# nextpyp/cet_pick

Hardware: AMD Instinct MI355X
Metric: subtomograms/sec (MoCo-3D train) + voxels/sec (heatmap+NMS) at 1/2/4/8 GPU (higher is better)
Workload: dtype f32; 1 GPU; moco_main.py moco3d_18: 3D encoder, synthetic 512x512x128 tomogram, 32^3 subtomo crops, batch 64 per GPU, r=1024, dim=128, m=0.999, T=0.1, SGD lr 1e-3; global_batch=64, parallelism=dp1, hipgraph=True

## Files before the change

cet_pick_amd/csrc/conv_direct3.hip:

```cpp
#include "common.h"
#include "bf16x3.h"
#include <type_traits>
#include <algorithm>

namespace {

using namespace bf3;

constexpr int C = 64;
constexpr int PLANE = 64;
constexpr int TZ = 2;
constexpr int PZ = TZ + 2;
constexpr int NV = PZ * PLANE;
constexpr int LEAD = 16;
constexpr int ZREC = 34;
constexpr int NREC = LEAD + NV + ZREC;
constexpr int ARR = NREC * 16;
constexpr int KS = C / 16;
constexpr int PL_BYTES = 2 * ARR;
constexpr int KS_BYTES = 3 * PL_BYTES;
constexpr int LDS_BYTES = KS * KS_BYTES;
constexpr int ZBASE = (LEAD + NV) * 16;
constexpr int WBLK = 1024;
constexpr int WSTEP = 2 * 3 * WBLK;
constexpr int NTAP = 27;
constexpr int NSTEP = KS * NTAP;
constexpr int WIMG_BYTES = NSTEP * WSTEP;
constexpr int RB = 6;
static_assert(NSTEP % RB == 0, "ring slots");
static_assert(LDS_BYTES <= 160 * 1024, "patch must fit the CU's LDS");
static_assert(((LEAD + NV) & 15) == 0, "zero region must start at a record = 0 (mod 16)");

struct Direct3Params {
    const float* a;
    const unsigned char* wimg;
    float* out;
    const float* res;
    const float* mask;
    int relu;
    int N, D;
    unsigned a_bytes;
};

template <bool TWO, int CT = C>
__global__ __launch_bounds__(256, TWO ? 2 : 1) void direct3_kernel(Direct3Params p) {
    constexpr int KS = CT / 16, NSTEP = KS * NTAP;
    constexpr int NSLOT = TWO ? 2 : KS;
    static_assert(NSTEP % RB == 0, "ring slots");
    __shared__ __attribute__((aligned(16))) unsigned char patch[NSLOT * KS_BYTES];
    const int tid = threadIdx.x, lane = tid & 63, wave = tid >> 6;
    const int h = lane >> 5, l32 = lane & 31;
    const int tz = wave >> 1, cw = wave & 1;
    const int zb = blockIdx.x % (p.D / TZ), n = blockIdx.x / (p.D / TZ);
    const int z0 = zb * TZ;

    const int cb = blockIdx.y;
    const __amdgpu_buffer_rsrc_t wrs = rsrc(p.wimg, (CT / 64) * NSTEP * WSTEP);
    const int w_voff = cw * (3 * WBLK) + lane * 16;
    const int w_cb = cb * (NSTEP * WSTEP);
    bf16x8 bfr[RB][3];
    auto wload = [&](int g, auto SLOTc) {
        constexpr int SLOT = decltype(SLOTc)::value;
#pragma unroll
        for (int pl = 0; pl < 3; ++pl)
            bfr[SLOT][pl] = __builtin_bit_cast(bf16x8, __builtin_amdgcn_raw_buffer_load_b128(wrs, g < NSTEP ? w_voff + pl * WBLK : (int)0x80000000u, g < NSTEP ? w_cb + g * WSTEP : 0, 0));
    };
    auto wload_dyn = [&](int g) {
        switch (g % RB) {
            case 0: wload(g, std::integral_constant<int, 0>{}); break;
            case 1: wload(g, std::integral_constant<int, 1>{}); break;
            case 2: wload(g, std::integral_constant<int, 2>{}); break;
            case 3: wload(g, std::integral_constant<int, 3>{}); break;
            case 4: wload(g, std::integral_constant<int, 4>{}); break;
            default: wload(g, std::integral_constant<int, 5>{}); break;
        }
    };
#pragma unroll
    for (int g = 0; g < RB - 1; ++g) wload_dyn(g);

    const __amdgpu_buffer_rsrc_t ars = rsrc(p.a, p.a_bytes);
    unsigned st_off[2];
    int st_lds[2];
#pragma unroll
    for (int u = 0; u < 2; ++u) {
        const int q = tid + 256 * u, vox = q >> 1, hh = q & 1;
        const int z = z0 - 1 + (vox >> 6);
        const bool ok = (unsigned)z < (unsigned)p.D;
        st_off[u] = ok ? 4u * (unsigned)((((long)n * p.D + z) * PLANE + (vox & 63)) * CT + hh * 8) : 0x80000000u;
        st_lds[u] = hh * ARR + (LEAD + vox) * 16;
    }
    u32x4 ld[2][2];
    auto stage_load = [&](int c) {
#pragma unroll
        for (int u = 0; u < 2; ++u) {
            ld[u][0] = __builtin_amdgcn_raw_buffer_load_b128(ars, (int)(st_off[u] + 64u * c), 0, 0);
            ld[u][1] = __builtin_amdgcn_raw_buffer_load_b128(ars, (int)(st_off[u] + 64u * c + 16u), 0, 0);
        }
    };
    auto stage_store = [&](int c) {
#pragma unroll
        for (int u = 0; u < 2; ++u) {
            float v[8];
#pragma unroll
            for (int e = 0; e < 4; ++e) { v[e] = __uint_as_float(ld[u][0][e]); v[4 + e] = __uint_as_float(ld[u][1][e]); }
            u32x4 o[3];
            cut8(v, o);
            unsigned char* dst = patch + (c % NSLOT) * KS_BYTES + st_lds[u];
#pragma unroll
            for (int pl = 0; pl < 3; ++pl) *reinterpret_cast<u32x4*>(dst + pl * PL_BYTES) = o[pl];
        }
    };
    stage_load(0);
    for (int i = tid; i < NSLOT * 3 * 2 * ZREC; i += 256) {
        const int arr = i / ZREC, r = i % ZREC;
        *reinterpret_cast<u32x4*>(patch + arr * ARR + ZBASE + r * 16) = u32x4{0u, 0u, 0u, 0u};
    }

    int vbase[2], zbase[2];
    unsigned vmask[2];
#pragma unroll
    for (int i = 0; i < 2; ++i) {
        const int y = 4 * i + (l32 >> 3), x = l32 & 7;
        const int rec = LEAD - 9 + tz * PLANE + y * 8 + x;
        vbase[i] = rec * 16 + h * ARR;
        zbase[i] = ZBASE + (rec & 15) * 16 + h * ARR;
        unsigned m = 0;
#pragma unroll
        for (int dy = 0; dy < 3; ++dy)
#pragma unroll
            for (int dx = 0; dx < 3; ++dx)
                if ((unsigned)(y + dy - 1) < 8u && (unsigned)(x + dx - 1) < 8u) m |= 1u << (dy * 3 + dx);
        vmask[i] = m;
    }

    f32x16 acc[2];
#pragma unroll
    for (int r = 0; r < 16; ++r) { acc[0][r] = 0.f; acc[1][r] = 0.f; }

    const long m0 = ((long)n * p.D + z0 + tz) * PLANE;
    const int col = cb * 64 + cw * 32 + l32;
    unsigned eoff[2][16];
    float rv[2][16], mv[2][16];
#pragma unroll
    for (int i = 0; i < 2; ++i)
#pragma unroll
        for (int r = 0; r < 16; ++r) eoff[i][r] = 4u * (unsigned)((m0 + 32 * i + (r & 3) + 8 * (r >> 2) + 4 * h) * CT + col);
    const __amdgpu_buffer_rsrc_t rrs = rsrc(p.res, p.res ? p.a_bytes : 0u), mrs = rsrc(p.mask, p.mask ? p.a_bytes : 0u);

    stage_store(0);
    stage_load(1);
    __syncthreads();

    bf16x8 af[2][2][3];
    int sel[9][2];
    auto make_sel = [&](int dz) {
#pragma unroll
        for (int t9 = 0; t9 < 9; ++t9)
#pragma unroll
            for (int i = 0; i < 2; ++i) sel[t9][i] = ((vmask[i] >> t9) & 1u) ? vbase[i] + dz * (PLANE * 16) : zbase[i];
    };
    auto frags = [&](int c, int t9, auto SETc) {
        constexpr int SET = decltype(SETc)::value;
        const int imm = ((t9 / 3) * 8 + (t9 % 3)) * 16 + (c % NSLOT) * KS_BYTES;
#pragma unroll
        for (int i = 0; i < 2; ++i)
#pragma unroll
            for (int pl = 0; pl < 3; ++pl)
                af[SET][i][pl] = *reinterpret_cast<const bf16x8*>(patch + sel[t9][i] + imm + pl * PL_BYTES);
    };
    auto frags_dyn = [&](int g, int c, int t9) {
        if (g & 1) frags(c, t9, std::integral_constant<int, 1>{});
        else frags(c, t9, std::integral_constant<int, 0>{});
    };

    make_sel(0);
    frags_dyn(0, 0, 0);
    __builtin_amdgcn_sched_barrier(0);
#pragma unroll
    for (int c = 0; c < KS; ++c) {
#pragma unroll
        for (int dz = 0; dz < 3; ++dz) {
#pragma unroll
            for (int t9 = 0; t9 < 9; ++t9) {
                const int g = c * NTAP + dz * 9 + t9;
                wload_dyn(g + RB - 1);
                if (dz == 1 && t9 == 0 && c + 1 < KS) {
                    stage_store(c + 1);
                    if (c + 2 < KS) stage_load(c + 2);
                }
                if (!TWO && c == KS - 1 && dz == 0 && t9 == 0) {
#pragma unroll
                    for (int i = 0; i < 2; ++i)
#pragma unroll
                        for (int r = 0; r < 16; ++r) {
                            rv[i][r] = __uint_as_float(__builtin_amdgcn_raw_buffer_load_b32(rrs, (int)eoff[i][r], 0, 0));
                            mv[i][r] = __uint_as_float(__builtin_amdgcn_raw_buffer_load_b32(mrs, (int)eoff[i][r], 0, 0));
                        }
                }
                if (g + 1 < NSTEP) {
                    const int c2 = (g + 1) / NTAP, r2 = (g + 1) % NTAP;
                    if (r2 == 0) __syncthreads();
                    if (r2 % 9 == 0) make_sel(r2 / 9);
                    frags_dyn(g + 1, c2, r2 % 9);
                }
#pragma unroll
                for (int pr = 0; pr < 6; ++pr) {
                    acc[0] = __builtin_amdgcn_mfma_f32_32x32x16_bf16(af[g & 1][0][PA[pr]], bfr[g % RB][PB[pr]], acc[0], 0, 0, 0);
                    acc[1] = __builtin_amdgcn_mfma_f32_32x32x16_bf16(af[g & 1][1][PA[pr]], bfr[g % RB][PB[pr]], acc[1], 0, 0, 0);
                }
#pragma unroll
                for (int k = 0; k < 6; ++k) {
                    __builtin_amdgcn_sched_group_barrier(0x008, 1, 0);
                    __builtin_amdgcn_sched_group_barrier(0x100, 1, 0);
                }
#pragma unroll
                for (int k = 0; k < 3; ++k) {
                    __builtin_amdgcn_sched_group_barrier(0x008, 1, 0);
                    __builtin_amdgcn_sched_group_barrier(0x020, 1, 0);
                }
                __builtin_amdgcn_sched_group_barrier(0x008, 3, 0);
                __builtin_amdgcn_sched_barrier(0);
            }
        }
    }

    const bool has_mask = p.mask != nullptr;
    if constexpr (TWO) {
#pragma unroll
        for (int i = 0; i < 2; ++i) {
            float rr[16], mm[16];
#pragma unroll
            for (int r = 0; r < 16; ++r) {
                const unsigned eo = 4u * (unsigned)((m0 + 32 * i + (r & 3) + 8 * (r >> 2) + 4 * h) * CT + col);
                rr[r] = __uint_as_float(__builtin_amdgcn_raw_buffer_load_b32(rrs, (int)eo, 0, 0));
                mm[r] = __uint_as_float(__builtin_amdgcn_raw_buffer_load_b32(mrs, (int)eo, 0, 0));
            }
#pragma unroll
            for (int r = 0; r < 16; ++r) {
                const unsigned eo = 4u * (unsigned)((m0 + 32 * i + (r & 3) + 8 * (r >> 2) + 4 * h) * CT + col);
                float v = acc[i][r] + rr[r];
                if (p.relu) v = fmaxf(v, 0.f);
                if (has_mask) v = (mm[r] > 0.f) ? v : 0.f;
                p.out[eo / 4] = v;
            }
        }
        return;
    }
#pragma unroll
    for (int i = 0; i < 2; ++i)
#pragma unroll
        for (int r = 0; r < 16; ++r) {
            float v = acc[i][r] + rv[i][r];
            if (p.relu) v = fmaxf(v, 0.f);
            if (has_mask) v = (mv[i][r] > 0.f) ? v : 0.f;
            p.out[eoff[i][r] / 4] = v;
        }
}

constexpr int HP = 10;
constexpr int H_NV = PZ * HP * HP;
constexpr int H_ARR = H_NV * 16;
constexpr int H_PL = 2 * H_ARR;
constexpr int H_KS = 3 * H_PL;
constexpr int H_UNITS = (2 * H_NV + 255) / 256;

struct Direct3hParams {
    const float* a;
    const unsigned char* wimg;
    float* out;
    const float* res;
    const float* mask;
    int relu;
    int N, D, H, W;
    unsigned a_bytes;
};

__global__ __launch_bounds__(256, 2) void direct3h_kernel(Direct3hParams p) {
    __shared__ __attribute__((aligned(16))) unsigned char patch[2 * H_KS];
    const int tid = threadIdx.x, lane = tid & 63, wave = tid >> 6;
    const int h = lane >> 5, l32 = lane & 31;
    const int tz = wave >> 1, cw = wave & 1;
    const int txn = (p.W + 7) / 8, tyn = (p.H + 7) / 8;
    int bi = blockIdx.x;
    const int bx = bi % txn; bi /= txn;
    const int by = bi % tyn; bi /= tyn;
    const int zb = bi % (p.D / TZ), n = bi / (p.D / TZ);
    const int z0 = zb * TZ, y0 = by * 8, x0 = bx * 8;

    const __amdgpu_buffer_rsrc_t wrs = rsrc(p.wimg, WIMG_BYTES);
    const int w_voff = cw * (3 * WBLK) + lane * 16;
    bf16x8 bfr[RB][3];
    auto wload = [&](int g, auto SLOTc) {
        constexpr int SLOT = decltype(SLOTc)::value;
#pragma unroll
        for (int pl = 0; pl < 3; ++pl)
            bfr[SLOT][pl] = __builtin_bit_cast(bf16x8, __builtin_amdgcn_raw_buffer_load_b128(wrs, g < NSTEP ? w_voff + pl * WBLK : (int)0x80000000u, g < NSTEP ? g * WSTEP : 0, 0));
    };
    auto wload_dyn = [&](int g) {
        switch (g % RB) {
            case 0: wload(g, std::integral_constant<int, 0>{}); break;
            case 1: wload(g, std::integral_constant<int, 1>{}); break;
            case 2: wload(g, std::integral_constant<int, 2>{}); break;
            case 3: wload(g, std::integral_constant<int, 3>{}); break;
            case 4: wload(g, std::integral_constant<int, 4>{}); break;
            default: wload(g, std::integral_constant<int, 5>{}); break;
        }
// ... 147 lines not shown
    constexpr int KSn = CT / 16;
    const int lane = idx & 63, cw = (idx >> 6) & 1, rest = idx >> 7, ks = rest % KSn, tap = (rest / KSn) % NTAP, cb = rest / (KSn * NTAP);
    if (cb >= CT / 64) return;
    const int nn = cb * 64 + cw * 32 + (lane & 31), k0 = ks * 16 + 8 * (lane >> 5);
    float v[8];
    if (dgrad) {
        ld8(w + ((long)(NTAP - 1 - tap) * CT + nn) * CT + k0, v);
    } else {
#pragma unroll
        for (int e = 0; e < 8; ++e) v[e] = w[((long)tap * CT + k0 + e) * CT + nn];
    }
    u32x4 o[3];
    cut8(v, o);
    unsigned char* dst = img + (long)(((cb * KSn + ks) * NTAP + tap) * 2 + cw) * (3 * WBLK) + lane * 16;
    store_planes(dst, WBLK, o);
}
__global__ __launch_bounds__(256) void direct3_prep_kernel(PrepBatch b) {
    const int fmt = b.wide[blockIdx.y], idx = blockIdx.x * 256 + threadIdx.x;
    if (fmt == 1) { if (blockIdx.x < PREP_BLOCKS_WIDE) direct3s_prep_body(b.w[blockIdx.y], b.img[blockIdx.y], b.dgrad[blockIdx.y], idx); }
    else if (fmt == 2) { if (blockIdx.x < PREP_BLOCKS_WIDE) direct3_prep_body<128>(b.w[blockIdx.y], b.img[blockIdx.y], b.dgrad[blockIdx.y], idx); }
    else if (fmt == 3) direct3s256_prep_body(b.w[blockIdx.y], b.img[blockIdx.y], b.dgrad[blockIdx.y], idx);
    else if (blockIdx.x < PREP_BLOCKS) direct3_prep_body<C>(b.w[blockIdx.y], b.img[blockIdx.y], b.dgrad[blockIdx.y], idx);
}

constexpr int WG_SPLITS = 28;
constexpr int WROW = 64;
constexpr int WHALF = (PLANE + 1) * WROW;
constexpr int WPL = 2 * WHALF;
constexpr int WOP = 3 * WPL;
constexpr int WBUF = 2 * WOP;
constexpr int WZERO = PLANE * WROW;

constexpr int WG_MAXPROB = 4;
struct Direct3WgradParams {
    const float* x[WG_MAXPROB];
    const float* dy[WG_MAXPROB];
    float* slabs[WG_MAXPROB];
    int N, D;
    unsigned bytes;
    int nprob, splits;
    int H, W;
};

constexpr int W_HB = 3 * 2 * 8 * 128;
template <bool V4, int CT, bool TILED = false>
__global__ __launch_bounds__(512, 2) void direct3_wgrad_kernel(Direct3WgradParams p) {
    __shared__ __attribute__((aligned(16))) unsigned char lds[2 * WBUF + (TILED ? 2 * W_HB : 16)];
    unsigned char* const halo = lds + 2 * WBUF;
    static_assert(!TILED || (!V4 && CT == 64), "tiled planes: the 64-channel geometry");
    constexpr int NBLK = CT / 64;
    const int tid = threadIdx.x, lane = tid & 63;
    const int wave = __builtin_amdgcn_readfirstlane(tid >> 6);
    const int h = lane >> 5, l32 = lane & 31, i16 = lane & 15, g16 = (lane >> 4) & 1;
    const int kh = wave >> 2, wm = (wave >> 1) & 1, wn = wave & 1;
    const int per_grp = p.nprob * p.splits;
    const int grp = blockIdx.x / per_grp, rem = blockIdx.x % per_grp;
    const int pb = rem / p.splits, split = rem % p.splits, stride = p.splits;
    const int pair = grp % 9, chb = grp / 9;
    const int ci0 = (chb / NBLK) * 64, co0 = (chb % NBLK) * 64;
    const int dz = pair / 3, dy = pair % 3;
    const int tiles_x = TILED ? p.W >> 3 : 1, tiles = TILED ? (p.H >> 3) * tiles_x : 1;
    const int n_planes = p.N * p.D * tiles;

    const __amdgpu_buffer_rsrc_t xrs = rsrc(p.x[pb], p.bytes), yrs = rsrc(p.dy[pb], p.bytes);
    const int st_vox = tid >> 3, st_cg = tid & 7;
    const unsigned st_src = TILED ? 4u * (unsigned)(((st_vox >> 3) * p.W + (st_vox & 7)) * C + st_cg * 8)
                                  : 4u * (unsigned)(st_vox * CT + st_cg * 8);
    const int h_side = tid >> 8, h_row = (tid >> 5) & 7, h_c2 = tid & 31;
    const unsigned x_ch = 4u * (unsigned)ci0, y_ch = 4u * (unsigned)co0;
    const int zsh = V4 ? 0 : dz - 1;
    const int st_lds = (st_cg >> 2) * WHALF + st_vox * WROW + (st_cg & 3) * 16;
    auto next_plane = [&](int from) {
        if (V4) return from < n_planes ? from : -1;
        for (int pi = from; pi < n_planes; pi += stride) {
            const int zi = (pi / tiles) % p.D + dz - 1;
            if ((unsigned)zi < (unsigned)p.D) return pi;
        }
        return -1;
    };
    u32x4 ldx[2], ldy[2];
    u32x2 ldh = {0u, 0u};
    unsigned u_y, u_x, u_h;
    auto unit_offsets = [&](int pi) {
        if (pi < 0) { u_y = u_x = u_h = 0x80000000u; return; }
        if (!TILED) {
            u_y = 4u * (unsigned)((long)pi * PLANE * CT) + y_ch + st_src;
            u_x = 4u * (unsigned)((long)(pi + zsh) * PLANE * CT) + x_ch + st_src;
            u_h = 0x80000000u;
            return;
        }
        const int pl = pi / tiles, t = pi % tiles, y0 = (t / tiles_x) * 8, x0 = (t % tiles_x) * 8;
        u_y = 4u * (unsigned)((((long)pl * p.H + y0) * p.W + x0) * C) + st_src;
        const int xr = y0 + (st_vox >> 3) + dy - 1;
        u_x = (unsigned)xr < (unsigned)p.H
                  ? 4u * (unsigned)((((long)(pl + dz - 1) * p.H + xr) * p.W + x0 + (st_vox & 7)) * C + st_cg * 8) : 0x80000000u;
        const int hr = y0 + h_row + dy - 1, hc = h_side ? x0 + 8 : x0 - 1;
        u_h = ((unsigned)hr < (unsigned)p.H && (unsigned)hc < (unsigned)p.W)
                  ? 4u * (unsigned)((((long)(pl + dz - 1) * p.H + hr) * p.W + hc) * C + 2 * h_c2) : 0x80000000u;
    };
    auto stage_load = [&](int pi) {
        unit_offsets(pi);
        ldx[0] = __builtin_amdgcn_raw_buffer_load_b128(xrs, (int)u_x, 0, 0);
        ldx[1] = __builtin_amdgcn_raw_buffer_load_b128(xrs, (int)(u_x + 16u), 0, 0);
        ldy[0] = __builtin_amdgcn_raw_buffer_load_b128(yrs, (int)u_y, 0, 0);
        ldy[1] = __builtin_amdgcn_raw_buffer_load_b128(yrs, (int)(u_y + 16u), 0, 0);
        if (TILED) ldh = __builtin_amdgcn_raw_buffer_load_b64(xrs, (int)u_h, 0, 0);
    };
    unsigned hcu[3];
    auto halo_cut = [&]() {
        const unsigned a1 = rest(ldh[0]), b1 = rest(ldh[1]), a2 = rest(a1), b2 = rest(b1);
        hcu[0] = pack2(ldh[1], ldh[0]);
        hcu[1] = pack2(b1, a1);
        hcu[2] = pack2(b2, a2);
    };
    auto halo_store = [&](int buf) {
#pragma unroll
        for (int pl = 0; pl < 3; ++pl)
            *reinterpret_cast<unsigned*>(halo + buf * W_HB + ((pl * 2 + h_side) * 8 + h_row) * 128 + h_c2 * 4) = hcu[pl];
    };
    auto stage_store_unit = [&](int buf, int op) {
        float v[8];
#pragma unroll
        for (int e = 0; e < 4; ++e) {
            v[e] = __uint_as_float(op ? ldy[0][e] : ldx[0][e]);
            v[4 + e] = __uint_as_float(op ? ldy[1][e] : ldx[1][e]);
        }
        u32x4 o[3];
        cut8(v, o);
        unsigned char* dst = lds + buf * WBUF + op * WOP + st_lds;
#pragma unroll
        for (int pl = 0; pl < 3; ++pl) *reinterpret_cast<u32x4*>(dst + pl * WPL) = o[pl];
        if (TILED && op == 0) { halo_cut(); halo_store(buf); }
    };

    const int q4 = i16 >> 2;
    const int coloff = (16 * g16 + 4 * (i16 & 3)) * 2;
    const int b_base = wn * WHALF + (2 * kh * 16 + 8 * h + q4) * WROW + coloff;
    int a_sel[2][2];
#pragma unroll
    for (int lk = 0; lk < 2; ++lk)
#pragma unroll
        for (int hi = 0; hi < 2; ++hi) {
            const int v = 16 * (2 * kh + lk) + 8 * h + 4 * hi + q4;
            if (V4) {
                const int zi = (v >> 4) + dz - 1, yi = ((v >> 2) & 3) + dy - 1;
                a_sel[lk][hi] = wm * WHALF + (((unsigned)zi < 4u && (unsigned)yi < 4u) ? ((zi * 4 + yi) * 4 + (v & 3)) * WROW : WZERO) + coloff;
            } else if (TILED) {
                a_sel[lk][hi] = wm * WHALF + v * WROW + coloff;
            } else {
                const int yi = (v >> 3) + dy - 1;
                a_sel[lk][hi] = wm * WHALF + ((unsigned)yi < 8u ? (yi * 8 + (v & 7)) * WROW : WZERO) + coloff;
            }
        }
    int h_off[2];
#pragma unroll
    for (int lk = 0; lk < 2; ++lk) h_off[lk] = (2 * (2 * kh + lk) + h) * 128 + (32 * wm + l32) * 2;
    unsigned hl[2][2][3];

    f32x16 acc[3];
#pragma unroll
    for (int t = 0; t < 3; ++t)
#pragma unroll
        for (int r = 0; r < 16; ++r) acc[t][r] = 0.f;

    for (int i = tid; i < 2 * 2 * 3 * 2 * (WROW / 16); i += 512) {
        const int img = i / (WROW / 16), c16 = i % (WROW / 16);
        *reinterpret_cast<u32x4*>(lds + img * WHALF + WZERO + c16 * 16) = u32x4{0u, 0u, 0u, 0u};
    }

    int cur = next_plane(split);
    int nxt = cur >= 0 ? next_plane(cur + stride) : -1;
    stage_load(cur);
    if (cur >= 0) { stage_store_unit(0, 0); stage_store_unit(0, 1); }
    stage_load(nxt);
    __syncthreads();

    bf16x8 af[2][3][3], bfg[2][3];
    auto read_piece = [&](int buf, int lk, int j, auto SETc) {
        constexpr int SET = decltype(SETc)::value;
        const unsigned char* xb = lds + buf * WBUF;
        if (j < 3) {
            const unsigned char* yb = xb + WOP + b_base + lk * 16 * WROW + j * WPL;
            const bf16x4 lo = __builtin_amdgcn_ds_read_tr16_b64_v4bf16((lds_bf16x4*)(yb));
            const bf16x4 hi = __builtin_amdgcn_ds_read_tr16_b64_v4bf16((lds_bf16x4*)(yb + 4 * WROW));
            bfg[SET][j] = __builtin_shufflevector(lo, hi, 0, 1, 2, 3, 4, 5, 6, 7);
        } else {
            const int pl = j - 3;
            const bf16x4 lo = __builtin_amdgcn_ds_read_tr16_b64_v4bf16((lds_bf16x4*)(xb + pl * WPL + a_sel[lk][0]));
            const bf16x4 hi = __builtin_amdgcn_ds_read_tr16_b64_v4bf16((lds_bf16x4*)(xb + pl * WPL + a_sel[lk][1]));
            af[SET][1][pl] = __builtin_shufflevector(lo, hi, 0, 1, 2, 3, 4, 5, 6, 7);
            if (TILED) {
#pragma unroll
                for (int sd = 0; sd < 2; ++sd)
                    hl[SET][sd][pl] = *reinterpret_cast<const unsigned short*>(halo + buf * W_HB + ((pl * 2 + sd) * 8) * 128 + h_off[lk]);
            }
        }
    };
    auto read_piece_dyn = [&](int buf, int lk, int j) {
        if (lk & 1) read_piece(buf, lk, j, std::integral_constant<int, 1>{});
        else read_piece(buf, lk, j, std::integral_constant<int, 0>{});
    };
    auto read_pair = [&](int buf, int lk, int i) {
        constexpr int BP[3] = {0, 2, 1}, AP[3] = {2, 0, 1};
        read_piece_dyn(buf, lk, BP[i]);
        read_piece_dyn(buf, lk, 3 + AP[i]);
    };
    auto derive = [&](int set, int dxv, int pl) {
        const u32x4 c = __builtin_bit_cast(u32x4, af[set][1][pl]);
        u32x4 o;
        if (dxv == 0) {
            o[0] = c[0] << 16;
#pragma unroll
            for (int j = 1; j < 4; ++j) o[j] = __builtin_amdgcn_alignbit(c[j], c[j - 1], 16);
            if (V4) o[2] &= HI16;
            if (TILED) o[0] |= hl[set][0][pl];
        } else {
#pragma unroll
            for (int j = 0; j < 3; ++j) o[j] = __builtin_amdgcn_alignbit(c[j + 1], c[j], 16);
            o[3] = c[3] >> 16;
            if (V4) o[1] &= 0x0000ffffu;
            if (TILED) o[3] |= hl[set][1][pl] << 16;
        }
        af[set][dxv][pl] = __builtin_bit_cast(bf16x8, o);
    };
    unsigned cu[3][8];
    auto cut_a = [&](int op, int e) {
        cu[0][e] = op ? ldy[e >> 2][e & 3] : ldx[e >> 2][e & 3];
        cu[1][e] = rest(cu[0][e]);
    };
    auto cut_b = [&](int e) { cu[2][e] = rest(cu[1][e]); };
    auto store_piece = [&](int buf, int op, int pl) {
        u32x4 o;
#pragma unroll
        for (int d = 0; d < 4; ++d) o[d] = pack2(cu[pl][2 * d + 1], cu[pl][2 * d]);
        *reinterpret_cast<u32x4*>(lds + buf * WBUF + op * WOP + st_lds + pl * WPL) = o;
    };

    int buf = 0;
    if (cur >= 0) {
#pragma unroll
        for (int i = 0; i < 3; ++i) read_pair(0, 0, i);
    }
    constexpr int DXO[3] = {1, 0, 2};
    while (cur >= 0) {
        const int nn = nxt >= 0 ? next_plane(nxt + stride) : -1;
        unit_offsets(nn);
        __builtin_amdgcn_sched_barrier(0);
#pragma unroll
        for (int lk = 0; lk < 2; ++lk) {
            const int op = lk;
#pragma unroll
            for (int m = 0; m < 18; ++m) {
                const int dxm = DXO[m / 6];
                acc[dxm] = __builtin_amdgcn_mfma_f32_32x32x16_bf16(af[lk][dxm][PA[m % 6]], bfg[lk][PB[m % 6]], acc[dxm], 0, 0, 0);
                if (m < 3) derive(lk, 0, m);
                if (m >= 6 && m < 9) derive(lk, 2, m - 6);
                if (m >= 2 && m < 10) cut_a(op, m - 2);
                if (m >= 3 && m < 11) cut_b(m - 3);
                if (m >= 11 && m < 14) store_piece(buf ^ 1, op, m - 11);
                if (lk == 1 && m >= 14) {
                    const int i = m - 14, hf = i & 1;
                    if (i < 2) ldx[hf] = __builtin_amdgcn_raw_buffer_load_b128(xrs, (int)(u_x + 16u * hf), 0, 0);
                    else ldy[hf] = __builtin_amdgcn_raw_buffer_load_b128(yrs, (int)(u_y + 16u * hf), 0, 0);
                    if (TILED && i == 3) ldh = __builtin_amdgcn_raw_buffer_load_b64(xrs, (int)u_h, 0, 0);
                }
                if (TILED && lk == 0 && m == 14) halo_cut();
                if (TILED && lk == 0 && m == 15) halo_store(buf ^ 1);
                if (lk == 0) {
                    if (m < 3) read_pair(buf, 1, m);
                } else {
                    if (m == 13) __syncthreads();
                    if (m >= 14 && m < 17 && nxt >= 0) read_pair(buf ^ 1, 0, m - 14);
                }
                __builtin_amdgcn_sched_barrier(0);
            }
        }
        buf ^= 1;
        cur = nxt;
        nxt = nn;
    }

    __syncthreads();
    float* red = reinterpret_cast<float*>(lds);
    if (kh == 1) {
#pragma unroll
        for (int dx = 0; dx < 3; ++dx)
#pragma unroll
            for (int r = 0; r < 16; ++r) red[(((wave & 3) * 3 + dx) * 16 + r) * 64 + lane] = acc[dx][r];
    }
    __syncthreads();
    if (kh == 1) return;
    float* out = p.slabs[pb] + (long)split * (NTAP * CT * CT);
#pragma unroll
    for (int dx = 0; dx < 3; ++dx) {
        const int tap = (dz * 3 + dy) * 3 + dx;
#pragma unroll
        for (int r = 0; r < 16; ++r) {
            const int ci = ci0 + 32 * wm + (r & 3) + 8 * (r >> 2) + 4 * h;
            out[((long)tap * CT + ci) * CT + co0 + 32 * wn + l32] = acc[dx][r] + red[((wave * 3 + dx) * 16 + r) * 64 + lane];
        }
    }
}

constexpr int CS = 128;
constexpr int VS = 64;
constexpr int S_LEAD = 32;
constexpr int S_NV = VS;
constexpr int S_ZREC = 64;
constexpr int S_NREC = S_LEAD + S_NV + S_ZREC;
constexpr int S_ARR = S_NREC * 16;
constexpr int S_PL = 2 * S_ARR;
constexpr int S_KS = 3 * S_PL;
constexpr int S_CH = 2 * S_KS;
constexpr int S_ZBASE = (S_LEAD + S_NV) * 16;
constexpr int S_CHUNKS = 4;
constexpr int S_LDS = S_CHUNKS * S_CH;
constexpr int S_STEPS = 2 * NTAP;
constexpr int S_WSTEP = 4 * 3 * WBLK;
constexpr int S_WIMG_BYTES = S_CHUNKS * S_STEPS * S_WSTEP;
static_assert(S_STEPS % RB == 0, "ring slots");
static_assert(((S_LEAD + S_NV) & 15) == 0, "zero region must start at a record = 0 (mod 16)");
static_assert(S_LDS <= 160 * 1024 && 4 * 32 * 64 * 4 <= S_LDS, "patch (and the four partial tiles behind it) fit the LDS");

struct Direct3sParams {
    const float* a;
    const unsigned char* wimg;
    float* out;
    const float* res;
    const float* mask;
    int relu;
    int N;
    unsigned a_bytes;
};

template <int CT>
__global__ __launch_bounds__(256, 1) void direct3s_kernel(Direct3sParams p) {
    constexpr int NCB = CT / 32;
    constexpr int NPASS = NCB / S_CHUNKS;
    constexpr int WST = NCB * 3 * WBLK;
    __shared__ __attribute__((aligned(16))) unsigned char patch[S_LDS];
    const int tid = threadIdx.x, lane = tid & 63;
    const int cc = __builtin_amdgcn_readfirstlane(tid >> 6);
    const int h = lane >> 5, l32 = lane & 31;
    const int ct = blockIdx.x % NCB, n0 = blockIdx.x / NCB;

    const __amdgpu_buffer_rsrc_t wrs = rsrc(p.wimg, NCB * S_STEPS * WST);
    const int w_voff = ct * (3 * WBLK) + lane * 16;
    int w_soff = cc * (S_STEPS * WST);
    bf16x8 bfr[RB][3];
    auto wload = [&](int g, auto SLOTc) {
        constexpr int SLOT = decltype(SLOTc)::value;
        const int vo = g < S_STEPS ? w_voff : (int)0x80000000u;
        const int so = g < S_STEPS ? w_soff + g * WST : 0;
#pragma unroll
        for (int pl = 0; pl < 3; ++pl)
            bfr[SLOT][pl] = __builtin_bit_cast(bf16x8, __builtin_amdgcn_raw_buffer_load_b128(wrs, vo + pl * WBLK, so, 0));
    };
    auto wload_dyn = [&](int g) {
        switch (g % RB) {
            case 0: wload(g, std::integral_constant<int, 0>{}); break;
            case 1: wload(g, std::integral_constant<int, 1>{}); break;
            case 2: wload(g, std::integral_constant<int, 2>{}); break;
            case 3: wload(g, std::integral_constant<int, 3>{}); break;
            case 4: wload(g, std::integral_constant<int, 4>{}); break;
            default: wload(g, std::integral_constant<int, 5>{}); break;
        }
    };
    const __amdgpu_buffer_rsrc_t ars = rsrc(p.a, p.a_bytes);
    for (int i = tid; i < 12 * S_CHUNKS * S_ZREC; i += 256) {
        const int arr = i / S_ZREC, r = i % S_ZREC;
        *reinterpret_cast<u32x4*>(patch + arr * S_ARR + S_ZBASE + r * 16) = u32x4{0u, 0u, 0u, 0u};
    }
    auto stage = [&](int pass) {
        u32x4 ld[4][2];
#pragma unroll
        for (int u = 0; u < 4; ++u) {
            const int q = tid + 256 * u, vox = q >> 4, cg = q & 15;
            const unsigned off = 4u * (unsigned)(((long)n0 * VS + vox) * CT + pass * 128 + cg * 8);
            ld[u][0] = __builtin_amdgcn_raw_buffer_load_b128(ars, (int)off, 0, 0);
            ld[u][1] = __builtin_amdgcn_raw_buffer_load_b128(ars, (int)(off + 16u), 0, 0);
        }
#pragma unroll
        for (int u = 0; u < 4; ++u) {
            const int q = tid + 256 * u, vox = q >> 4, cg = q & 15;
            float v[8];
#pragma unroll
            for (int e = 0; e < 4; ++e) { v[e] = __uint_as_float(ld[u][0][e]); v[4 + e] = __uint_as_float(ld[u][1][e]); }
            u32x4 o[3];
            cut8(v, o);
            unsigned char* dst = patch + (cg >> 2) * S_CH + ((cg >> 1) & 1) * S_KS + (cg & 1) * S_ARR + (S_LEAD + vox) * 16;
#pragma unroll
            for (int pl = 0; pl < 3; ++pl) *reinterpret_cast<u32x4*>(dst + pl * S_PL) = o[pl];
        }
    };

    int vbase[2], zbase[2];
    unsigned vmask[2];
#pragma unroll
    for (int i = 0; i < 2; ++i) {
        const int v = 32 * i + l32, z = v >> 4, y = (v >> 2) & 3, x = v & 3;
        const int rec = S_LEAD - 21 + v;
        vbase[i] = cc * S_CH + rec * 16 + h * S_ARR;
        zbase[i] = cc * S_CH + S_ZBASE + (rec & 15) * 16 + h * S_ARR;
        unsigned m = 0;
#pragma unroll
        for (int t = 0; t < NTAP; ++t) {
            const int dz = t / 9, dy = (t / 3) % 3, dx = t % 3;
            if ((unsigned)(z + dz - 1) < 4u && (unsigned)(y + dy - 1) < 4u && (unsigned)(x + dx - 1) < 4u) m |= 1u << t;
        }
        vmask[i] = m;
    }

    f32x16 acc[2];
#pragma unroll
    for (int r = 0; r < 16; ++r) { acc[0][r] = 0.f; acc[1][r] = 0.f; }

    bf16x8 af[2][2][3];
    auto frags = [&](int g, auto SETc) {
        constexpr int SET = decltype(SETc)::value;
        const int tap = g >> 1, ksx = g & 1;
        const int imm = ((tap / 9) * 16 + ((tap / 3) % 3) * 4 + tap % 3) * 16 + ksx * S_KS;
#pragma unroll
        for (int i = 0; i < 2; ++i) {
            const int sel = ((vmask[i] >> tap) & 1u) ? vbase[i] : zbase[i];
#pragma unroll
            for (int pl = 0; pl < 3; ++pl)
                af[SET][i][pl] = *reinterpret_cast<const bf16x8*>(patch + sel + imm + pl * S_PL);
        }
    };
    auto frags_dyn = [&](int g) {
        if (g & 1) frags(g, std::integral_constant<int, 1>{});
        else frags(g, std::integral_constant<int, 0>{});
    };

#pragma unroll
    for (int pass = 0; pass < NPASS; ++pass) {
        w_soff = (pass * S_CHUNKS + cc) * (S_STEPS * WST);
        if (pass > 0) __syncthreads();
#pragma unroll
        for (int g = 0; g < RB - 1; ++g) wload_dyn(g);
        stage(pass);
        __syncthreads();
        frags_dyn(0);
        __builtin_amdgcn_sched_barrier(0);
    #pragma unroll
        for (int g = 0; g < S_STEPS; ++g) {
            wload_dyn(g + RB - 1);
            if (g + 1 < S_STEPS) frags_dyn(g + 1);
    #pragma unroll
            for (int pr = 0; pr < 6; ++pr) {
                acc[0] = __builtin_amdgcn_mfma_f32_32x32x16_bf16(af[g & 1][0][PA[pr]], bfr[g % RB][PB[pr]], acc[0], 0, 0, 0);
                acc[1] = __builtin_amdgcn_mfma_f32_32x32x16_bf16(af[g & 1][1][PA[pr]], bfr[g % RB][PB[pr]], acc[1], 0, 0, 0);
            }
    #pragma unroll
            for (int k = 0; k < 6; ++k) {
                __builtin_amdgcn_sched_group_barrier(0x008, 1, 0);
                __builtin_amdgcn_sched_group_barrier(0x100, 1, 0);
            }
    #pragma unroll
            for (int k = 0; k < 3; ++k) {
                __builtin_amdgcn_sched_group_barrier(0x008, 1, 0);
                __builtin_amdgcn_sched_group_barrier(0x020, 1, 0);
            }
            __builtin_amdgcn_sched_group_barrier(0x008, 3, 0);
            __builtin_amdgcn_sched_barrier(0);
        }
    }

    __syncthreads();
    float* red = reinterpret_cast<float*>(patch);
#pragma unroll
    for (int i = 0; i < 2; ++i)
#pragma unroll
        for (int r = 0; r < 16; ++r) red[(cc * 32 + i * 16 + r) * 64 + lane] = acc[i][r];
    __syncthreads();
    const long m0 = (long)n0 * VS;
    const int col = ct * 32 + l32;
#pragma unroll
    for (int j = 0; j < 8; ++j) {
        const int idx = cc * 8 + j, i = idx >> 4, r = idx & 15;
        float t = ((red[idx * 64 + lane] + red[(32 + idx) * 64 + lane]) + red[(64 + idx) * 64 + lane]) + red[(96 + idx) * 64 + lane];
        const long o = (m0 + 32 * i + (r & 3) + 8 * (r >> 2) + 4 * h) * CT + col;
        if (p.res) t += p.res[o];
        if (p.relu) t = fmaxf(t, 0.f);
        if (p.mask) t = (p.mask[o] > 0.f) ? t : 0.f;
        p.out[o] = t;
    }
}

template <int CT>
__device__ void direct3s_prep_body_t(const float* w, unsigned char* img, int dgrad, int idx) {
    constexpr int NCB = CT / 32;
    const int lane = idx & 63, cb = (idx >> 6) % NCB, r1 = (idx >> 6) / NCB, ksx = r1 & 1, rest = r1 >> 1, tap = rest % NTAP, cc = rest / NTAP;
    if (cc >= NCB) return;
    const int nn = cb * 32 + (lane & 31), k0 = cc * 32 + ksx * 16 + 8 * (lane >> 5);
    float v[8];
    if (dgrad) {
        ld8(w + ((long)(NTAP - 1 - tap) * CT + nn) * CT + k0, v);
    } else {
#pragma unroll
        for (int e = 0; e < 8; ++e) v[e] = w[((long)tap * CT + k0 + e) * CT + nn];
    }
    u32x4 o[3];
    cut8(v, o);
    unsigned char* dst = img + (long)(((cc * NTAP + tap) * 2 + ksx) * NCB + cb) * (3 * WBLK) + lane * 16;
    store_planes(dst, WBLK, o);
}
__device__ void direct3s_prep_body(const float* w, unsigned char* img, int dgrad, int idx) { direct3s_prep_body_t<CS>(w, img, dgrad, idx); }
__device__ void direct3s256_prep_body(const float* w, unsigned char* img, int dgrad, int idx) { direct3s_prep_body_t<256>(w, img, dgrad, idx); }

}

int mi_direct3_kind(int N, int Di, int Hi, int Wi, int Ci, int Co, int kd, int kh, int kw, int stride, int pd, int ph,
                    int pw, int dd, int dh, int dw) {
    const char* off = getenv("MI_CONV_NO_DIRECT");
    if (off && atoi(off) != 0) return 0;
    if (kd != 3 || kh != 3 || kw != 3 || stride != 1 || pd != 1 || ph != 1 || pw != 1 || dd != 1 || dh != 1 || dw != 1) return 0;
    if (N < 1 || 4l * N * Di * Hi * Wi * Ci >= 0x7fff0000l) return 0;
    if (Ci == C && Co == C && Hi == 8 && Wi == 8 && Di >= TZ && Di % TZ == 0) return 1;
    if (Ci == CS && Co == CS && Di == 4 && Hi == 4 && Wi == 4) return 2;
    if (Ci == 128 && Co == 128 && Hi == 8 && Wi == 8 && Di >= TZ && Di % TZ == 0 && (long)N * Di >= 128 && (long)N * (Di / TZ) <= 0x7fffffffl) return 3;
    if (Ci == 256 && Co == 256 && Di == 4 && Hi == 4 && Wi == 4 && N >= 16) return 4;
    if (Ci == C && Co == C && (Hi > 8 || Wi > 8) && Hi >= 8 && Wi >= 8 && Di >= TZ && Di % TZ == 0) {
        const bool ragged = Hi % 8 != 0 || Wi % 8 != 0;
        const char* rg = getenv("MI_DIRECT3H_RAGGED");
        const long ty = (Hi + 7) / 8, tx = (Wi + 7) / 8, wgs = (long)N * (Di / TZ) * ty * tx;
        const bool fill_ok = 4l * Hi * Wi >= 3l * 64 * ty * tx;
        const bool take = !ragged || (rg ? atoi(rg) != 0 : fill_ok);
        if (wgs >= 128 && wgs <= 0x7fffffffl && take) return 5;
    }
    return 0;
}
bool mi_direct3_usable(int N, int Di, int Hi, int Wi, int Ci, int Co, int kd, int kh, int kw, int stride, int pd, int ph,
                       int pw, int dd, int dh, int dw) {
    return mi_direct3_kind(N, Di, Hi, Wi, Ci, Co, kd, kh, kw, stride, pd, ph, pw, dd, dh, dw) != 0;
}

size_t mi_direct3_wimg_bytes(int channels) {
    return channels == C ? (size_t)WIMG_BYTES : channels == CS ? (size_t)S_WIMG_BYTES : 0;
}
size_t mi_direct3_wimg_bytes_kind(int kind) {
    return (kind == 1 || kind == 5) ? (size_t)WIMG_BYTES : kind == 2 ? (size_t)S_WIMG_BYTES : kind == 3 ? (size_t)(2 * 8 * NTAP * WSTEP)
         : kind == 4 ? (size_t)8 * S_STEPS * (8 * 3 * WBLK) : 0;
}
size_t mi_direct3_slab_bytes(int, int) { return 0; }

int mi_direct3_prep_kind(const float* const* w, void* const* img, const int* dgrad, const int* kinds, int n, hipStream_t s) {
    for (int i0 = 0; i0 < n; i0 += PREP_MAX) {
        PrepBatch b = {};
        const int m = n - i0 < PREP_MAX ? n - i0 : PREP_MAX;
        int blocks = PREP_BLOCKS;
        for (int i = 0; i < m; ++i) {
            const int kd = kinds[i0 + i];
            if (kd < 1 || kd > 5 || !w[i0 + i] || !img[i0 + i]) return MI_E_ARG;
            b.w[i] = w[i0 + i]; b.img[i] = (unsigned char*)img[i0 + i]; b.dgrad[i] = dgrad[i0 + i];
            b.wide[i] = kd == 5 ? 0 : kd - 1;
            blocks = std::max(blocks, kd == 4 ? PREP_BLOCKS_256 : (kd == 2 || kd == 3) ? PREP_BLOCKS_WIDE : PREP_BLOCKS);
        }
        hipLaunchKernelGGL(direct3_prep_kernel, dim3(blocks, m), dim3(256), 0, s, b);
        MI_RETURN_IF_LAUNCH_FAILED();
    }
    return MI_OK;
}
int mi_direct3_prep(const float* const* w, void* const* img, const int* dgrad, const int* channels, int n, hipStream_t s) {
    if (n > 4096) return MI_E_ARG;
    int kinds[4096];
    for (int i = 0; i < n; ++i) {
        if (channels[i] != C && channels[i] != CS) return MI_E_ARG;
        kinds[i] = channels[i] == C ? 1 : 2;
    }
    return mi_direct3_prep_kind(w, img, dgrad, kinds, n, s);
}

int mi_direct3_launch(const float* a, const void* wimg, float* out, const float* res, const float* mask, int relu, int N,
                      int D, hipStream_t s) {
    Direct3Params p = {a, (const unsigned char*)wimg, out, res, mask, relu, N, D, (unsigned)(4l * N * D * PLANE * C)};
    if (getenv("MI_DIRECT3_FOUR_SLOTS")) hipLaunchKernelGGL(direct3_kernel<false>, dim3((unsigned)(N * (D / TZ))), dim3(256), 0, s, p);
    else hipLaunchKernelGGL(direct3_kernel<true>, dim3((unsigned)(N * (D / TZ))), dim3(256), 0, s, p);
    MI_RETURN_IF_LAUNCH_FAILED();
    return MI_OK;
}
int mi_direct3h_launch(const float* a, const void* wimg, float* out, const float* res, const float* mask, int relu, int N,
                       int D, int H, int W, hipStream_t s) {
    Direct3hParams p = {a, (const unsigned char*)wimg, out, res, mask, relu, N, D, H, W, (unsigned)(4l * N * D * H * W * C)};
    hipLaunchKernelGGL(direct3h_kernel, dim3((unsigned)((long)N * (D / TZ) * ((H + 7) / 8) * ((W + 7) / 8))), dim3(256), 0, s, p);
    MI_RETURN_IF_LAUNCH_FAILED();
    return MI_OK;
}
int mi_direct3_launch128(const float* a, const void* wimg, float* out, const float* res, const float* mask, int relu, int N,
                         int D, hipStream_t s) {
    Direct3Params p = {a, (const unsigned char*)wimg, out, res, mask, relu, N, D, (unsigned)(4l * N * D * PLANE * 128)};
    hipLaunchKernelGGL((direct3_kernel<true, 128>), dim3((unsigned)(N * (D / TZ)), 2), dim3(256), 0, s, p);
    MI_RETURN_IF_LAUNCH_FAILED();
    return MI_OK;
}

int mi_direct3s_launch(const float* a, const void* wimg, float* out, const float* res, const float* mask, int relu, int N,
                       hipStream_t s) {
    Direct3sParams p = {a, (const unsigned char*)wimg, out, res, mask, relu, N, (unsigned)(4l * N * VS * CS)};
    hipLaunchKernelGGL(direct3s_kernel<CS>, dim3((unsigned)(4 * N)), dim3(256), 0, s, p);
    MI_RETURN_IF_LAUNCH_FAILED();
    return MI_OK;
}
int mi_direct3s_launch256(const float* a, const void* wimg, float* out, const float* res, const float* mask, int relu, int N,
                          hipStream_t s) {
    Direct3sParams p = {a, (const unsigned char*)wimg, out, res, mask, relu, N, (unsigned)(4l * N * VS * 256)};
    hipLaunchKernelGGL(direct3s_kernel<256>, dim3((unsigned)(8 * N)), dim3(256), 0, s, p);
    MI_RETURN_IF_LAUNCH_FAILED();
    return MI_OK;
}

size_t mi_direct3_wgrad_slab_bytes() { return sizeof(float) * (size_t)WG_SPLITS * NTAP * C * C; }
int mi_direct3_wgrad_splits() { return WG_SPLITS; }

int mi_direct3_wgrad_launch(const float* x, const float* dy, float* slabs, int N, int D, hipStream_t s) {
    Direct3WgradParams p = {};
    p.x[0] = x; p.dy[0] = dy; p.slabs[0] = slabs; p.N = N; p.D = D; p.bytes = (unsigned)(4l * N * D * PLANE * C);
    p.nprob = 1; p.splits = WG_SPLITS;
    hipLaunchKernelGGL((direct3_wgrad_kernel<false, 64>), dim3(9 * WG_SPLITS), dim3(512), 0, s, p);
    MI_RETURN_IF_LAUNCH_FAILED();
    return MI_OK;
}
int mi_direct3_wgrad_batch_max() { return WG_MAXPROB; }
constexpr int WG_BATCH_SPLITS = 7;
int mi_direct3_wgrad_batch_splits(int nb) {
    if (nb < 1 || nb > WG_MAXPROB) return 0;
    if (const char* v = getenv("MI_D3W_BATCH_SPLITS")) { const int sv = atoi(v); if (sv >= 1 && sv <= WG_SPLITS) return sv; }
    return WG_BATCH_SPLITS;
}
int mi_direct3_wgrad_launch_batch(const float* const* xs, const float* const* dys, float* const* slabs, int nb, int N, int D,
                                  hipStream_t s) {
    if (nb < 1 || nb > WG_MAXPROB) return MI_E_ARG;
    Direct3WgradParams p = {};
    for (int i = 0; i < nb; ++i) { p.x[i] = xs[i]; p.dy[i] = dys[i]; p.slabs[i] = slabs[i]; }
    p.N = N; p.D = D; p.bytes = (unsigned)(4l * N * D * PLANE * C);
    p.nprob = nb; p.splits = mi_direct3_wgrad_batch_splits(nb);
    hipLaunchKernelGGL((direct3_wgrad_kernel<false, 64>), dim3(9 * nb * p.splits), dim3(512), 0, s, p);
    MI_RETURN_IF_LAUNCH_FAILED();
    return MI_OK;
}

constexpr int WS_SPLITS = 7, WS_BATCH_SPLITS = 2;
size_t mi_direct3s_wgrad_slab_bytes() { return sizeof(float) * (size_t)WS_SPLITS * NTAP * CS * CS; }
int mi_direct3s_wgrad_splits(int nb) {
    if (nb < 1 || nb > WG_MAXPROB) return 0;
    if (nb == 1) return WS_SPLITS;
    if (const char* v = getenv("MI_D3SW_BATCH_SPLITS")) { const int sv = atoi(v); if (sv >= 1 && sv <= WS_SPLITS) return sv; }
    return WS_BATCH_SPLITS;
}
int mi_direct3s_wgrad_launch_batch(const float* const* xs, const float* const* dys, float* const* slabs, int nb, int N, hipStream_t s) {
    if (nb < 1 || nb > WG_MAXPROB || N < 1) return MI_E_ARG;
    Direct3WgradParams p = {};
    for (int i = 0; i < nb; ++i) { p.x[i] = xs[i]; p.dy[i] = dys[i]; p.slabs[i] = slabs[i]; }
    p.N = N; p.D = 1; p.bytes = (unsigned)(4l * N * PLANE * CS);
    p.nprob = nb; p.splits = mi_direct3s_wgrad_splits(nb);
    hipLaunchKernelGGL((direct3_wgrad_kernel<true, 128>), dim3(36 * nb * p.splits), dim3(512), 0, s, p);
    MI_RETURN_IF_LAUNCH_FAILED();
    return MI_OK;
}

int mi_direct3t_wgrad_launch(const float* x, const float* dy, float* slabs, int N, int D, int H, int W, hipStream_t s) {
    if (H % 8 || W % 8 || H < 8 || W < 8) return MI_E_UNSUPPORTED;
    Direct3WgradParams p = {};
    p.x[0] = x; p.dy[0] = dy; p.slabs[0] = slabs; p.N = N; p.D = D; p.H = H; p.W = W;
    p.bytes = (unsigned)(4l * N * D * H * W * C);
    p.nprob = 1; p.splits = WG_SPLITS;
    hipLaunchKernelGGL((direct3_wgrad_kernel<false, 64, true>), dim3(9 * WG_SPLITS), dim3(512), 0, s, p);
    MI_RETURN_IF_LAUNCH_FAILED();
    return MI_OK;
}

int mi_direct3x_wgrad_splits(int kind) { return kind == 3 ? 7 : 0; }
size_t mi_direct3x_wgrad_slab_bytes(int kind) {
    const size_t ct = kind == 3 ? 128 : 0;
    return sizeof(float) * (size_t)mi_direct3x_wgrad_splits(kind) * NTAP * ct * ct;
}
int mi_direct3x_wgrad_launch(int kind, const float* x, const float* dy, float* slabs, int N, int D, hipStream_t s) {
    Direct3WgradParams p = {};
    p.x[0] = x; p.dy[0] = dy; p.slabs[0] = slabs; p.nprob = 1; p.splits = mi_direct3x_wgrad_splits(kind);
    if (kind == 3) {
        p.N = N; p.D = D; p.bytes = (unsigned)(4l * N * D * PLANE * 128);
        hipLaunchKernelGGL((direct3_wgrad_kernel<false, 128>), dim3(36 * p.splits), dim3(512), 0, s, p);
    } else return MI_E_UNSUPPORTED;
    MI_RETURN_IF_LAUNCH_FAILED();
    return MI_OK;
}

int mi_direct3_finish_slabs(const float* slabs, int n_slabs, long out_elems, float* out, const float* res, const float* mask,
                            int relu, hipStream_t s);

extern "C" size_t mi_conv3d_direct_wimg_bytes(int channels) { return mi_direct3_wimg_bytes(channels); }
extern "C" size_t mi_conv3d_direct_workspace_bytes(int N, int channels) { return mi_direct3_slab_bytes(N, channels); }

extern "C" int mi_conv3d_direct_usable(int N, int Di, int Hi, int Wi, int Ci, int Co, int k, int stride, int pad) {
    const int kind = mi_direct3_kind(N, Di, Hi, Wi, Ci, Co, k, k, k, stride, pad, pad, pad, 1, 1, 1);
    return kind <= 2 ? kind : 0;
}

extern "C" int mi_conv3d_direct_prep(const void* const* w, void* const* img, const int* dgrad, const int* channels, int n,
                                     mi_stream_t stream) {
    if (!w || !img || !dgrad || !channels || n < 0) return MI_E_ARG;
    if (n == 0) return MI_OK;
    return mi_direct3_prep(reinterpret_cast<const float* const*>(w), img, dgrad, channels, n, (hipStream_t)stream);
}

extern "C" int mi_conv3d_direct_f32(const float* a, const void* wimg, float* out, const float* res, const float* mask,
                                    int relu, int N, int Di, int Hi, int Wi, int channels, void* ws, size_t ws_bytes,
                                    mi_stream_t stream) {
    if (!a || !wimg || !out) return MI_E_ARG;
    const int kind = mi_direct3_kind(N, Di, Hi, Wi, channels, channels, 3, 3, 3, 1, 1, 1, 1, 1, 1, 1);
    if (kind == 1) return mi_direct3_launch(a, wimg, out, res, mask, relu, N, Di, (hipStream_t)stream);
    if (kind == 2) return mi_direct3s_launch(a, wimg, out, res, mask, relu, N, (hipStream_t)stream);
    return MI_E_UNSUPPORTED;
}
```

Baseline: 40960 subtomograms/sec.

## Switch 4^3 direct conv to 16x16x32 MFMA tiles and skip dead z-planes

Rewrites the small-volume (4x4x4, 128/256-channel) direct 3D conv kernel to use 16x16x32 bf16 MFMAs over four 16-voxel row groups instead of two 32x32x16 tiles. Each row group is one z-plane, so taps whose z offset falls outside the volume can skip both their LDS fragment loads and their MFMAs at compile time. The weight image layout and the epilogue index mapping change to match the new tiling. The weight prefetch ring is now scheduled per tap, and the out-of-range load guard is removed. This adds more, smaller MFMA instructions and depends on the new sched_group_barrier counts matching the instruction mix.

```diff
diff --git a/cet_pick_amd/csrc/conv_direct3.hip b/cet_pick_amd/csrc/conv_direct3.hip
--- a/cet_pick_amd/csrc/conv_direct3.hip
+++ b/cet_pick_amd/csrc/conv_direct3.hip
@@ -2,6 +2,7 @@
 #include "bf16x3.h"
 #include <type_traits>
 #include <algorithm>
+#include <utility>
 
 namespace {
 
@@ -755,6 +756,15 @@
     }
 }
 
+#ifndef MI_DIRECT3S_ZSKIP
+#define MI_DIRECT3S_ZSKIP 1
+#endif
+constexpr bool S_ZSKIP = MI_DIRECT3S_ZSKIP != 0;
+typedef float f32x4 __attribute__((ext_vector_type(4)));
+constexpr bool s_zdead(int i, int tap) { return (i == 0 && tap / 9 == 0) || (i == 3 && tap / 9 == 2); }
+constexpr int s_live(int tap) { return S_ZSKIP && tap / 9 != 1 ? 3 : 4; }
+template <int... T, class F>
+__device__ __forceinline__ void s_for_each(std::integer_sequence<int, T...>, F&& f) { (f(std::integral_constant<int, T>{}), ...); }
 constexpr int CS = 128;
 constexpr int VS = 64;
 constexpr int S_LEAD = 32;
@@ -771,7 +781,7 @@
 constexpr int S_STEPS = 2 * NTAP;
 constexpr int S_WSTEP = 4 * 3 * WBLK;
 constexpr int S_WIMG_BYTES = S_CHUNKS * S_STEPS * S_WSTEP;
-static_assert(S_STEPS % RB == 0, "ring slots");
+static_assert(S_STEPS % RB == 0 && RB == 6, "ring slots: three taps of two fragments");
 static_assert(((S_LEAD + S_NV) & 15) == 0, "zero region must start at a record = 0 (mod 16)");
 static_assert(S_LDS <= 160 * 1024 && 4 * 32 * 64 * 4 <= S_LDS, "patch (and the four partial tiles behind it) fit the LDS");
 
@@ -794,7 +804,7 @@
     __shared__ __attribute__((aligned(16))) unsigned char patch[S_LDS];
     const int tid = threadIdx.x, lane = tid & 63;
     const int cc = __builtin_amdgcn_readfirstlane(tid >> 6);
-    const int h = lane >> 5, l32 = lane & 31;
+    const int kq = lane >> 4, l16 = lane & 15;
     const int ct = blockIdx.x % NCB, n0 = blockIdx.x / NCB;
 
     const __amdgpu_buffer_rsrc_t wrs = rsrc(p.wimg, NCB * S_STEPS * WST);
@@ -803,11 +813,9 @@
     bf16x8 bfr[RB][3];
     auto wload = [&](int g, auto SLOTc) {
         constexpr int SLOT = decltype(SLOTc)::value;
-        const int vo = g < S_STEPS ? w_voff : (int)0x80000000u;
-        const int so = g < S_STEPS ? w_soff + g * WST : 0;
 #pragma unroll
         for (int pl = 0; pl < 3; ++pl)
-            bfr[SLOT][pl] = __builtin_bit_cast(bf16x8, __builtin_amdgcn_raw_buffer_load_b128(wrs, vo + pl * WBLK, so, 0));
+            bfr[SLOT][pl] = __builtin_bit_cast(bf16x8, __builtin_amdgcn_raw_buffer_load_b128(wrs, w_voff + pl * WBLK, w_soff + g * WST, 0));
     };
     auto wload_dyn = [&](int g) {
         switch (g % RB) {
@@ -847,43 +855,46 @@
         }
     };
 
-    int vbase[2], zbase[2];
-    unsigned vmask[2];
-#pragma unroll
-    for (int i = 0; i < 2; ++i) {
-        const int v = 32 * i + l32, z = v >> 4, y = (v >> 2) & 3, x = v & 3;
-        const int rec = S_LEAD - 21 + v;
-        vbase[i] = cc * S_CH + rec * 16 + h * S_ARR;
-        zbase[i] = cc * S_CH + S_ZBASE + (rec & 15) * 16 + h * S_ARR;
-        unsigned m = 0;
-#pragma unroll
-        for (int t = 0; t < NTAP; ++t) {
-            const int dz = t / 9, dy = (t / 3) % 3, dx = t % 3;
-            if ((unsigned)(z + dz - 1) < 4u && (unsigned)(y + dy - 1) < 4u && (unsigned)(x + dx - 1) < 4u) m |= 1u << t;
-        }
-        vmask[i] = m;
-    }
-
-    f32x16 acc[2];
-#pragma unroll
-    for (int r = 0; r < 16; ++r) { acc[0][r] = 0.f; acc[1][r] = 0.f; }
-
-    bf16x8 af[2][2][3];
-    auto frags = [&](int g, auto SETc) {
+    const int qarr = cc * S_CH + (kq >> 1) * S_KS + (kq & 1) * S_ARR;
+    const int rec0 = S_LEAD - 21 + l16;
+    const int zbase = qarr + S_ZBASE + (rec0 & 15) * 16;
+    int vb[4];
+#pragma unroll
+    for (int i = 0; i < 4; ++i) vb[i] = qarr + (rec0 + 16 * i) * 16;
+    unsigned m9 = 0;
+    {
+        const int y = l16 >> 2, x = l16 & 3;
+#pragma unroll
+        for (int dy = 0; dy < 3; ++dy)
+#pragma unroll
+            for (int dx = 0; dx < 3; ++dx)
+                if ((unsigned)(y + dy - 1) < 4u && (unsigned)(x + dx - 1) < 4u) m9 |= 1u << (dy * 3 + dx);
+    }
+
+    f32x4 acc[4][2];
+#pragma unroll
+    for (int i = 0; i < 4; ++i)
+#pragma unroll
+        for (int j = 0; j < 2; ++j) acc[i][j] = f32x4{0.f, 0.f, 0.f, 0.f};
+
+    bf16x8 af[2][4][3];
+    auto frags = [&](int tap, auto SETc) {
         constexpr int SET = decltype(SETc)::value;
-        const int tap = g >> 1, ksx = g & 1;
-        const int imm = ((tap / 9) * 16 + ((tap / 3) % 3) * 4 + tap % 3) * 16 + ksx * S_KS;
-#pragma unroll
-        for (int i = 0; i < 2; ++i) {
-            const int sel = ((vmask[i] >> tap) & 1u) ? vbase[i] : zbase[i];
+        const int t9 = tap % 9;
+        const int imm = ((tap / 9) * 16 + (t9 / 3) * 4 + t9 % 3) * 16;
+        const bool in = (m9 >> t9) & 1u;
+#pragma unroll
+        for (int i = 0; i < 4; ++i) {
+            if (S_ZSKIP && s_zdead(i, tap)) continue;
+            const int sel = s_zdead(i, tap) ? zbase : (in ? vb[i] : zbase);
 #pragma unroll
             for (int pl = 0; pl < 3; ++pl)
                 af[SET][i][pl] = *reinterpret_cast<const bf16x8*>(patch + sel + imm + pl * S_PL);
         }
     };
-    auto frags_dyn = [&](int g) {
-        if (g & 1) frags(g, std::integral_constant<int, 1>{});
-        else frags(g, std::integral_constant<int, 0>{});
+    auto frags_dyn = [&](int tap) {
+        if (tap & 1) frags(tap, std::integral_constant<int, 1>{});
+        else frags(tap, std::integral_constant<int, 0>{});
     };
 
 #pragma unroll
@@ -891,49 +902,56 @@
         w_soff = (pass * S_CHUNKS + cc) * (S_STEPS * WST);
         if (pass > 0) __syncthreads();
 #pragma unroll
-        for (int g = 0; g < RB - 1; ++g) wload_dyn(g);
+        for (int g = 0; g < RB - 2; ++g) wload_dyn(g);
         stage(pass);
         __syncthreads();
         frags_dyn(0);
         __builtin_amdgcn_sched_barrier(0);
+        s_for_each(std::make_integer_sequence<int, NTAP>{}, [&](auto TAPc) {
+            constexpr int tap = decltype(TAPc)::value;
+            if (tap + 2 < NTAP) { wload_dyn(2 * tap + RB - 2); wload_dyn(2 * tap + RB - 1); }
+            if (tap + 1 < NTAP) frags_dyn(tap + 1);
     #pragma unroll
-        for (int g = 0; g < S_STEPS; ++g) {
-            wload_dyn(g + RB - 1);
-            if (g + 1 < S_STEPS) frags_dyn(g + 1);
+            for (int pr = 0; pr < 6; ++pr)
     #pragma unroll
-            for (int pr = 0; pr < 6; ++pr) {
-                acc[0] = __builtin_amdgcn_mfma_f32_32x32x16_bf16(af[g & 1][0][PA[pr]], bfr[g % RB][PB[pr]], acc[0], 0, 0, 0);
-                acc[1] = __builtin_amdgcn_mfma_f32_32x32x16_bf16(af[g & 1][1][PA[pr]], bfr[g % RB][PB[pr]], acc[1], 0, 0, 0);
-            }
+                for (int i = 0; i < 4; ++i) {
+                    if (S_ZSKIP && s_zdead(i, tap)) continue;
     #pragma unroll
-            for (int k = 0; k < 6; ++k) {
-                __builtin_amdgcn_sched_group_barrier(0x008, 1, 0);
+                    for (int j = 0; j < 2; ++j)
+                        acc[i][j] = __builtin_amdgcn_mfma_f32_16x16x32_bf16(af[tap & 1][i][PA[pr]], bfr[(2 * tap + j) % RB][PB[pr]], acc[i][j], 0, 0, 0);
+                }
+            constexpr int n_lds = tap + 1 < NTAP ? 3 * s_live(tap + 1) : 0, n_vm = tap + 2 < NTAP ? 6 : 0;
+    #pragma unroll
+            for (int k = 0; k < n_lds; ++k) {
+                __builtin_amdgcn_sched_group_barrier(0x008, 2, 0);
                 __builtin_amdgcn_sched_group_barrier(0x100, 1, 0);
             }
     #pragma unroll
-            for (int k = 0; k < 3; ++k) {
-                __builtin_amdgcn_sched_group_barrier(0x008, 1, 0);
+            for (int k = 0; k < n_vm; ++k) {
+                __builtin_amdgcn_sched_group_barrier(0x008, 2, 0);
                 __builtin_amdgcn_sched_group_barrier(0x020, 1, 0);
             }
-            __builtin_amdgcn_sched_group_barrier(0x008, 3, 0);
+    #pragma unroll
+            for (int k = 2 * (n_lds + n_vm); k < 12 * s_live(tap); ++k) __builtin_amdgcn_sched_group_barrier(0x008, 1, 0);
             __builtin_amdgcn_sched_barrier(0);
-        }
+        });
     }
 
     __syncthreads();
     float* red = reinterpret_cast<float*>(patch);
 #pragma unroll
-    for (int i = 0; i < 2; ++i)
-#pragma unroll
-        for (int r = 0; r < 16; ++r) red[(cc * 32 + i * 16 + r) * 64 + lane] = acc[i][r];
+    for (int i = 0; i < 4; ++i)
+#pragma unroll
+        for (int j = 0; j < 2; ++j)
+#pragma unroll
+            for (int r = 0; r < 4; ++r) red[(cc * 32 + (i * 2 + j) * 4 + r) * 64 + lane] = acc[i][j][r];
     __syncthreads();
-    const long m0 = (long)n0 * VS;
-    const int col = ct * 32 + l32;
-#pragma unroll
-    for (int j = 0; j < 8; ++j) {
-        const int idx = cc * 8 + j, i = idx >> 4, r = idx & 15;
+    const long m0 = (long)n0 * VS + 16 * cc + 4 * kq;
+#pragma unroll
+    for (int jr = 0; jr < 8; ++jr) {
+        const int idx = cc * 8 + jr, j = jr >> 2, r = jr & 3;
         float t = ((red[idx * 64 + lane] + red[(32 + idx) * 64 + lane]) + red[(64 + idx) * 64 + lane]) + red[(96 + idx) * 64 + lane];
-        const long o = (m0 + 32 * i + (r & 3) + 8 * (r >> 2) + 4 * h) * CT + col;
+        const long o = (m0 + r) * CT + ct * 32 + j * 16 + l16;
         if (p.res) t += p.res[o];
         if (p.relu) t = fmaxf(t, 0.f);
         if (p.mask) t = (p.mask[o] > 0.f) ? t : 0.f;
@@ -944,9 +962,9 @@
 template <int CT>
 __device__ void direct3s_prep_body_t(const float* w, unsigned char* img, int dgrad, int idx) {
     constexpr int NCB = CT / 32;
-    const int lane = idx & 63, cb = (idx >> 6) % NCB, r1 = (idx >> 6) / NCB, ksx = r1 & 1, rest = r1 >> 1, tap = rest % NTAP, cc = rest / NTAP;
+    const int lane = idx & 63, cb = (idx >> 6) % NCB, r1 = (idx >> 6) / NCB, jt = r1 & 1, rest = r1 >> 1, tap = rest % NTAP, cc = rest / NTAP;
     if (cc >= NCB) return;
-    const int nn = cb * 32 + (lane & 31), k0 = cc * 32 + ksx * 16 + 8 * (lane >> 5);
+    const int nn = cb * 32 + jt * 16 + (lane & 15), k0 = cc * 32 + 8 * (lane >> 4);
     float v[8];
     if (dgrad) {
         ld8(w + ((long)(NTAP - 1 - tap) * CT + nn) * CT + k0, v);
@@ -956,7 +974,7 @@
     }
     u32x4 o[3];
     cut8(v, o);
-    unsigned char* dst = img + (long)(((cc * NTAP + tap) * 2 + ksx) * NCB + cb) * (3 * WBLK) + lane * 16;
+    unsigned char* dst = img + (long)(((cc * NTAP + tap) * 2 + jt) * NCB + cb) * (3 * WBLK) + lane * 16;
     store_planes(dst, WBLK, o);
 }
 __device__ void direct3s_prep_body(const float* w, unsigned char* img, int dgrad, int idx) { direct3s_prep_body_t<CS>(w, img, dgrad, idx); }
```

New measurement: 41590 subtomograms/sec, median of 6. +1.6%, better.
